# regeirk/pycwt

Hardware: NVIDIA H100
Metric: cwt_scale_points_per_sec (higher is better)
Workload: dtype f64

## Files before the change

### pycwt_b200/csrc/engine.cu

```cuda
#include <algorithm>
#include <array>
#include <cmath>
#include <cstdint>
#include <cstdio>
#include <cstdlib>
#include <cstring>
#include <map>
#include <mutex>
#include <set>
#include <string>
#include <type_traits>
#include <vector>

#include <cuda_runtime.h>
#include <dlfcn.h>
#include <initializer_list>

#include "../../include/cwt_b200.h"
#include "kernels.cuh"

using namespace cwtb;

template <class B, class = void> struct BodyNT { static constexpr int value = NT; };
template <class B> struct BodyNT<B, std::void_t<decltype(B::NTB)>> { static constexpr int value = B::NTB; };
// ... 100 lines not shown
  int log2K;
  int first, count;
  int expand = 0;
  int log2Nc = 0;
  int taps = 0;
  long long woff = 0;
  int os = 0;
};

struct ResidentSlot {
  Buf buf;
  int S = 0;
  long long n0 = 0;
  int prec = 0;
  long long serial = 0;
  Buf counts;
  long long units = -1;
};

static void slot_begin(ResidentSlot &s) {
  ++s.serial;
  s.S = 0;
  s.n0 = 0;
  s.units = -1;
}

struct OsRow { int grp = 0, t1 = 0, M = 0; long long hoff = 0; };

struct Job {
  bool valid = false;
  int precision = 0;
  long long n0 = 0;
  unsigned N = 0;
  int log2N = 0;
  int S = 0;
  int nbatch = 1;
  double dt = 0;
  Fam fam{};
  std::vector<ScaleDesc> descs;
  std::vector<ClassRun> classes;
  std::vector<int> plan_log2K;
  std::vector<double> scales;
  size_t b_single = 0;
  size_t coarse_elems = 0;
  int sig_is_f32 = 0;
  bool exact = false;
  std::vector<OsGroup> os_groups;
};

struct BluePlan {
  unsigned n = 0, L = 0;
  double2 *wm = nullptr;
  double2 *bf[2] = {nullptr, nullptr};
};

struct NTabDev {
  double2 *hi = nullptr, *lo = nullptr;
  int h = 0;
};

struct cwtb_ctx {
  int device = 0;
  rt_stream stream{};
  rt_stream aux_stream{};
  rt_stream prio_stream{};
  rt_stream prio_short{};
  int prio_mode = 1;
  rt_stream chain_streams[3]{};
  int n_chains = 2;
  rt_stream cur{};
  int pad_pow2 = 1;
  int coh_precision = 0;
  std::map<unsigned, BluePlan> blue;
  rt_stream copy_streams[2]{};
  std::string err;
  double band_eps = 1e-16;
  double band_eps32 = 1e-9;
  double expand_eps = 5e-13;
  double expand_eps32 = 2e-7;
  int expand_mma = 1;
  int dense_margin = 2;
  int expand_min_log2R = 0;
  int os_on = 1;
  Buf osH, osgrp;
  void *comm = nullptr;
  int comm_world = 1, comm_rank = 0;
  Buf comm_send, comm_recv;
  int group = 0;
  size_t group_bytes = (size_t)512 << 20;
  int num_sms = 132;
  int pf_dist = 132;
  int pf_rows_a = 32, pf_rows_b = 32;
  int pf_dist_a = 132;
  size_t batch_bytes = (size_t)4 << 30;
  double2 *tw64 = nullptr;
  float2 *tw32 = nullptr;
  std::map<unsigned, NTabDev> ntabs;
  Buf filt;
  int filt_rows = 0;
  long long filt_n = 0;
  Buf Zx, Cout, wtab;
  std::map<std::array<long long, 3>, long long> wtab_index;
  std::vector<double> wtab_host;
  size_t wtab_uploaded = 0;
  size_t wtab_max_bytes = (size_t)256 << 20;
  Buf sig, sig2, sig3, spec, Z, Zc[3], Y, B, W, W2, W3, descs, table, scratch, C, A12, F, aux, rowd, win, mask, hist, noise, wide, blueA, blueX, blueY, pspec, prot;
  Job job;
  struct PlanKey {
    long long n0 = -1;
    double dt = 0, param = 0, band_eps = 0, band_eps32 = 0, expand_eps = 0, expand_eps32 = 0;
    int S = 0, family = 0, precision = 0, nbatch = 0, pad = 0;
    std::vector<double> scales;
    bool operator==(const PlanKey &o) const {
      return n0 == o.n0 && dt == o.dt && param == o.param && band_eps == o.band_eps && band_eps32 == o.band_eps32 &&
             expand_eps == o.expand_eps && expand_eps32 == o.expand_eps32 && S == o.S && family == o.family &&
             precision == o.precision && nbatch == o.nbatch && pad == o.pad && scales == o.scales;
    }
  } plan_key;
  int plan_reuse = 1;
  void *stage_host[2] = {nullptr, nullptr};
  size_t stage_bytes = 0;
  Buf stage_dev[2], batch_power;
  int batch_pipeline = 1;
  double *angle_host = nullptr;
  ResidentSlot coh;
  ResidentSlot cross;
  ResidentSlot coh3;
  ResidentSlot wt;
  const void *job_dsig = nullptr;
  double last_ms = 0;
  int launches = 0;
  std::set<const void *> configured;
  bool profiling = false;
  const char *prof_tag = "";
  struct ProfRec { std::string name; unsigned gx, gy; int ev; };
  std::vector<ProfRec> prof;
  std::vector<rt_event> prof_events;
  std::set<void *> pinned, devallocs;
  rt_event e0{}, e1{};
  rt_event ev_fork{}, ev_join{}, ev_joinc[3]{}, ev_coarse{}, ev_coarse_short{};
  rt_event ev_h2d[2]{}, ev_used[2]{};
  rt_event ev_angle{};
};

static int fail(cwtb_ctx *c, int code, const std::string &msg) {
  if (c) c->err = msg;
  return code;
}
#define RT(call)                                                                             \
  do {                                                                                       \
    int e_ = (call);                                                                         \
    if (e_ != 0) return fail(c, CWTB_ERR_CUDA, std::string(#call) + ": " + rt_errstr(e_));   \
  } while (0)

static int ensure(cwtb_ctx *c, Buf &b, size_t bytes) {
  if (b.bytes >= bytes && b.p) return 0;
  if (b.p) rt_free(b.p);
  b.p = nullptr;
  b.bytes = 0;
  if (rt_malloc(&b.p, bytes) != 0) return fail(c, CWTB_ERR_NOMEM, "device allocation failed");
  b.bytes = bytes;
  return 0;
}

#ifdef CWTB_HOST_EMU
template <class Body, int PH>
static void emu_phases(const typename Body::Args &a, int bx, int by, void *sm) {
  for (int tid = 0; tid < BodyNT<Body>::value; ++tid) Body::template phase<PH>(a, bx, by, tid, sm);
  if constexpr (PH + 1 < Body::NPHASE) emu_phases<Body, PH + 1>(a, bx, by, sm);
}
#endif

static std::string body_name(const char *pretty) {
  std::string s(pretty);
  size_t i = s.find("Body = ");
  if (i == std::string::npos) return s;
  s = s.substr(i + 7);
  size_t j = s.find_first_of(";]");
  if (j != std::string::npos) s = s.substr(0, j);
  if (s.rfind("cwtb::", 0) == 0) s = s.substr(6);
  return s;
}

constexpr unsigned MAX_ROWS = 65535;

template <class Body, class Dispatch>
static int launch_rec(cwtb_ctx *c, unsigned gx, unsigned gy, Dispatch &&dispatch) {
  if (gx == 0 || gy == 0) return 0;
  if (gy > MAX_ROWS) return fail(c, CWTB_ERR_ARG, "too many rows in one launch");
  int ev = -1;
  if (c->profiling) {
    ev = (int)c->prof.size() * 2;
    while ((int)c->prof_events.size() < ev + 2) {
      rt_event e;
      RT(rt_event_create(&e));
      c->prof_events.push_back(e);
    }
    c->prof.push_back({std::string(c->prof_tag) + body_name(__PRETTY_FUNCTION__), gx, gy, ev});
    RT(rt_record(c->prof_events[ev], c->cur));
  }
  int e = dispatch();
  if (e) return e;
  if (ev >= 0) RT(rt_record(c->prof_events[ev + 1], c->cur));
  c->launches++;
  return 0;
}

template <class Body>
static int launch(cwtb_ctx *c, unsigned gx, unsigned gy, const typename Body::Args &a) {
  return launch_rec<Body>(c, gx, gy, [&]() -> int {
#ifdef CWTB_HOST_EMU
    std::vector<unsigned char> smv(Body::SMEM + 64);
    unsigned char *sm = smv.data();
    sm += (16 - ((unsigned long long)sm & 15)) & 15;
    for (unsigned by = 0; by < gy; ++by)
      for (unsigned bx = 0; bx < gx; ++bx) emu_phases<Body, 0>(a, (int)bx, (int)by, sm);
    if (emu_bulk_copy_faults() != 0) {
      emu_bulk_copy_faults() = 0;
      return fail(c, CWTB_ERR_CUDA, "emulation: bulk-async copy with a misaligned address or size");
    }
#else
    const void *fn = (const void *)k_run<Body>;
    if (Body::SMEM > 48 * 1024 && !c->configured.count(fn)) {
// ... 550 lines not shown
  for (int r0 = 0; r0 < nrows; r0 += chunk) {
    const int nr = std::min(chunk, nrows - r0);
    BluePreArgs pa{(const char *)in + (size_t)r0 * in_pitch * isz, (double2 *)c->blueA.p, pl->wm,
                   in_pitch, (long long)n, n, real_in, sign};
    if ((e = launch<BluePreBody>(c, (n + NT - 1) / NT, nr, pa))) return e;
    if ((e = blue_convolve(c, *pl, nr, sign))) return e;
    BluePostArgs po{(const double2 *)c->blueY.p, out, pl->wm, nullptr, out_pitch, nout,
                    scale / (double)pl->L, pl->L, 0, r0, sign, EPI_STORE};
    if ((e = launch<BluePostBody>(c, (unsigned)((nout + NT - 1) / NT), nr, po))) return e;
  }
  return 0;
}

static int run_job_exact(cwtb_ctx *c, const Job &job, const double *dsig, double2 *Wout, int epi) {
  const unsigned n = job.N;
  const int S = job.S;
  int e;
  if (job.nbatch != 1) return fail(c, CWTB_ERR_UNSUPPORTED, "batched transforms need the padded mode");
  if ((e = ensure(c, c->spec, (size_t)n * sizeof(double2)))) return e;
  if (!Wout) {
    if ((e = ensure(c, c->W, (size_t)S * job.n0 * sizeof(double2)))) return e;
    Wout = (double2 *)c->W.p;
  }
  if ((e = blue_rows(c, dsig, 1, n, (double2 *)c->spec.p, n, n, 1, -1, 1.0, n))) return e;
  const BluePlan *pl;
  if ((e = get_blue(c, n, &pl))) return e;
  Fam fam = job.fam;
  if (fam.family == CWTB_TABLE) fam.table = (const double2 *)c->table.p;
  const int chunk = blue_chunk_rows(pl->L, S);
  if ((e = ensure(c, c->blueA, (size_t)chunk * n * sizeof(double2)))) return e;
  if ((e = ensure(c, c->blueX, (size_t)chunk * pl->L * sizeof(double2)))) return e;
  if ((e = ensure(c, c->blueY, (size_t)chunk * pl->L * sizeof(double2)))) return e;
  const ScaleDesc *ddesc = (const ScaleDesc *)c->descs.p;
  for (int r0 = 0; r0 < S; r0 += chunk) {
    const int nr = std::min(chunk, S - r0);
    BlueProdArgs pa{ddesc, (const double2 *)c->spec.p, (double2 *)c->blueA.p, pl->wm, fam, (long long)n, n, r0};
    if ((e = launch<BlueProdBody>(c, (n + NT - 1) / NT, nr, pa))) return e;
    if ((e = blue_convolve(c, *pl, nr, +1))) return e;
    BluePostArgs po{(const double2 *)c->blueY.p, Wout, pl->wm, ddesc, job.n0, job.n0,
                    1.0 / (double)pl->L, pl->L, r0, 0, +1, epi};
    if ((e = launch<BluePostBody>(c, (unsigned)((job.n0 + NT - 1) / NT), nr, po))) return e;
  }
  return 0;
}

template <typename T, int K>
static int launch_single(cwtb_ctx *c, const SingleArgs<T> &a, int count) {
  constexpr int P = Lay<T, K>::P;
  const unsigned M = a.N / K;
  return launch<SingleBody<T, K>>(c, (M + P - 1) / P, count, a);
}

static int chunk_rows(const cwtb_ctx *c, unsigned N, size_t elem_bytes) {
  if (c->group > 0) return c->group;
  size_t g = c->group_bytes / ((size_t)N * elem_bytes);
  return (int)std::max<size_t>(1, std::min<size_t>(g, 32768));
}

static bool class_single(const Job &job, const ClassRun &cl) {
  return !cl.expand && !cl.os && (cl.log2K <= 10 || (cl.log2K <= DIRECT_MAX_LOG2 && cl.log2K < job.log2N));
}
static bool class_two_kernel(const Job &job, const ClassRun &cl) {
  return !cl.expand && !cl.os && !class_single(job, cl);
}

static int job_chain_region(const cwtb_ctx *c, const Job &job, const ClassRun &cl) {
  int idx = 0;
  for (const ClassRun &o : job.classes) {
    if (&o == &cl) break;
    if (class_two_kernel(job, o)) ++idx;
  }
  return idx % std::max(1, c->n_chains);
}

static size_t band_chunk_elems(const Job &job, int G) {
  size_t bchunk = 0;
  for (const ClassRun &cl : job.classes)
    if (class_two_kernel(job, cl) && cl.log2K < job.log2N)
      bchunk = std::max(bchunk, (size_t)std::min(G, cl.count) << cl.log2K);
  return bchunk;
}

#ifndef CWTB_HOST_EMU
template <class Body>
static int launch_persistent(cwtb_ctx *c, unsigned gm, unsigned rows, const typename Body::Args &a) {
  auto kern = k_persist<Body>;
  const void *fn = (const void *)kern;
  if (!c->configured.count(fn)) {
    RT(cudaFuncSetAttribute(kern, cudaFuncAttributeMaxDynamicSharedMemorySize, (int)Body::SMEM));
    c->configured.insert(fn);
  }
  int occ = 0;
  RT(cudaOccupancyMaxActiveBlocksPerMultiprocessor(&occ, kern, Body::NTB, Body::SMEM));
  if (occ < 1) return fail(c, CWTB_ERR_CUDA, "persistent kernel does not fit on an SM");
  const unsigned long long total = (unsigned long long)gm * rows;
  if (total > 0xffffffffull) return fail(c, CWTB_ERR_ARG, "too many tiles in one launch");
  const unsigned grid = (unsigned)std::min<unsigned long long>(total, (unsigned long long)occ * c->num_sms);
  return launch_rec<Body>(c, grid, rows, [&]() -> int {
    kern<<<grid, Body::NTB, Body::SMEM, c->cur>>>(a, gm, (unsigned)total);
    RT(cudaGetLastError());
    return 0;
  });
}
#endif

template <class Body, typename T>
static int launch_coarse(cwtb_ctx *c, CoarseArgs<T> a, const std::vector<CoarseSeg> &segs) {
  for (size_t s0 = 0; s0 < segs.size(); s0 += CSEG_MAX) {
    a.nseg = (int)std::min<size_t>(CSEG_MAX, segs.size() - s0);
    unsigned ctas = 0;
    for (int i = 0; i < a.nseg; ++i) {
      a.seg[i] = segs[s0 + i];
      a.seg[i].cta0 = (int)ctas;
      ctas += (unsigned)Body::ctas(a.seg[i].log2Nc, a.seg[i].count);
    }
    int e = launch<Body>(c, ctas, 1, a);
    if (e) return e;
  }
  return 0;
}

template <typename T, int TAPS>
static int launch_expand_t(cwtb_ctx *c, const ExpandArgs<T> &a, int rows, int min_log2Nc) {
  using B = ExpandBody<T, TAPS>;
  const unsigned gx = std::max<unsigned>(1, a.N / (unsigned)(B::NT * B::L));
#ifndef CWTB_HOST_EMU
  if constexpr (std::is_same<T, double>::value) {
    static_assert(ExpandMmaBody<TAPS>::OUT_PER_CTA == 4096, "the planner assumes the tensor-core kernel from Np = 2^12");
    if (c->expand_mma && a.N >= (unsigned)ExpandMmaBody<TAPS>::OUT_PER_CTA) {
      const unsigned gm = a.N / (32u * std::min<unsigned>(ExpandMmaBody<TAPS>::L, 1u << min_log2Nc));
      if (a.epi == EPI_MULCONJ) return launch_persistent<ExpandMmaBody<TAPS, EPI_MULCONJ>>(c, gm, rows, a);
      return launch_persistent<ExpandMmaBody<TAPS>>(c, gm, rows, a);
    }
  }
  if constexpr (TAPS > 16) {
    return fail(c, CWTB_ERR_STATE, "expansion: tap counts above 16 exist on the tensor-core kernel only");
  } else
#endif
  {
    if (a.epi == EPI_MULCONJ) return launch<ExpandBody<T, TAPS, EPI_MULCONJ>>(c, gx, rows, a);
    return launch<B>(c, gx, rows, a);
  }
}
template <typename T>
static int launch_expand(cwtb_ctx *c, int taps, const ExpandArgs<T> &a, int rows, int min_log2Nc) {
  if constexpr (std::is_same<T, double>::value) {
    switch (taps) {
      case 10: return launch_expand_t<T, 10>(c, a, rows, min_log2Nc);
      case 12: return launch_expand_t<T, 12>(c, a, rows, min_log2Nc);
      case 14: return launch_expand_t<T, 14>(c, a, rows, min_log2Nc);
      case 16: return launch_expand_t<T, 16>(c, a, rows, min_log2Nc);
      case 20: return launch_expand_t<T, 20>(c, a, rows, min_log2Nc);
    }
  } else {
    switch (taps) {
      case 6: return launch_expand_t<T, 6>(c, a, rows, min_log2Nc);
      case 8: return launch_expand_t<T, 8>(c, a, rows, min_log2Nc);
      case 10: return launch_expand_t<T, 10>(c, a, rows, min_log2Nc);
    }
  }
  return fail(c, CWTB_ERR_STATE, "expansion: unsupported tap count");
}

template <typename T>
static int run_job(cwtb_ctx *c, const Job &job, const T *dsig, cx<T> *Wout = nullptr, int epi = EPI_STORE) {
  using V = cx<T>;
  if (job.exact) {
    if constexpr (std::is_same<T, double>::value) return run_job_exact(c, job, dsig, Wout, epi);
    else return fail(c, CWTB_ERR_UNSUPPORTED, "un-padded transforms run in fp64");
  }
  const unsigned N = job.N;
  const int S = job.S * job.nbatch;
  int e;
  struct CurGuard { cwtb_ctx *c; ~CurGuard() { c->cur = c->stream; c->prof_tag = ""; } } cur_guard{c};
  if ((e = ensure(c, c->spec, (size_t)job.nbatch * N * sizeof(V)))) return e;
  if (!Wout) {
    if ((e = ensure(c, c->W, (size_t)S * job.n0 * sizeof(V)))) return e;
    Wout = (V *)c->W.p;
  }
  V *spec = (V *)c->spec.p;
  V *W = Wout;
  const ScaleDesc *ddesc = (const ScaleDesc *)c->descs.p;
  Fam fam = job.fam;
  if (fam.family == CWTB_TABLE) fam.table = (const double2 *)c->table.p;

  if (N < 32) {
    if (job.nbatch != 1) return fail(c, CWTB_ERR_UNSUPPORTED, "batched transform needs n0 > 16");
    TinyFwdArgs<T> fa{dsig, spec, job.n0, N};
    if ((e = launch<TinyFwdBody<T>>(c, 1, 1, fa))) return e;
    TinyArgs<T> ta{ddesc, spec, W, fam, job.n0, N, 0, epi};
    return launch<TinyBody<T>>(c, (unsigned)((job.n0 + NT - 1) / NT), S, ta);
  }
  c->prof_tag = "fwd:";
  e = fft_rows<T, -1>(c, dsig, 1, job.n0, job.n0, spec, N, N, job.nbatch);
  c->prof_tag = "";
  if (e) return e;

  NTab nt;
  if ((e = get_ntab(c, N, job.log2N, &nt))) return e;
  const int G = chunk_rows(c, N, sizeof(V));
  const size_t bchunk = band_chunk_elems(job, G);
  if ((e = ensure(c, c->B, (job.b_single + (size_t)std::max(1, c->n_chains) * bchunk) * sizeof(V)))) return e;
  V *Bbuf = (V *)c->B.p;

  {
    int first = -1, maxlk = 0, nrows = 0;
    for (const ClassRun &cl : job.classes)
      if (class_single(job, cl)) {
        if (first < 0) first = cl.first;
        maxlk = std::max(maxlk, cl.log2K);
        nrows += cl.count;
      }
    if (first >= 0) {
      BandArgs<T> ba{ddesc, spec, Bbuf, fam, N, first};
      const unsigned Kmax = 1u << maxlk;
      if ((e = launch<BandBody<T>>(c, (Kmax + NT * BandBody<T>::PER - 1) / (NT * BandBody<T>::PER), nrows, ba)))
        return e;
    }
  }
  const bool split = !c->profiling;
  if (split) {
    RT(rt_record(c->ev_fork, c->stream));
    RT(rt_wait(c->aux_stream, c->ev_fork));
    for (int k = 1; k < c->n_chains; ++k) RT(rt_wait(c->chain_streams[k - 1], c->ev_fork));
  }
  if (job.coarse_elems) {
    const bool prio = split && c->prio_mode > 0;
    if (prio) {
      RT(rt_wait(c->prio_stream, c->ev_fork));
      RT(rt_wait(c->prio_short, c->ev_fork));
    }
    if (split) c->cur = prio ? c->prio_stream : c->aux_stream;
    if ((e = ensure(c, c->Cout, job.coarse_elems * sizeof(V)))) return e;
    std::vector<CoarseSeg> short_segs, long_segs;
    size_t zx_elems = 0;
    for (size_t ci = 0; ci < job.classes.size(); ++ci) {
      const ClassRun &cl = job.classes[ci];
      if (!cl.expand) continue;
      if (cl.log2Nc < 6 || cl.log2Nc > 20)
        return fail(c, CWTB_ERR_STATE, "expansion: coarse length outside 2^6 .. 2^20");
      std::vector<CoarseSeg> &v = cl.log2Nc <= 10 ? short_segs : long_segs;
      if (ci > 0 && job.classes[ci - 1].expand && job.classes[ci - 1].log2Nc == cl.log2Nc) v.back().count += cl.count;
      else v.push_back(CoarseSeg{cl.first, cl.count, cl.log2Nc, 0});
      if (cl.log2Nc > 10)
        zx_elems = std::max(zx_elems, (size_t)job.descs[cl.first].ip_coff + ((size_t)cl.count << cl.log2Nc));
    }
    CoarseArgs<T> ca{};
    ca.descs = ddesc; ca.spec = spec; ca.C = (V *)c->Cout.p; ca.tw = Tw<T>::get(c); ca.fam = fam; ca.Nx = N;
    ca.pf_dist = c->pf_rows_b;
    c->prof_tag = "coarse:";
    if (!long_segs.empty()) {
      if ((e = ensure(c, c->Zx, zx_elems * sizeof(V)))) return e;
      ca.Z = (V *)c->Zx.p;
      for (const CoarseSeg &g : long_segs)
        if ((e = get_ntab(c, 1u << g.log2Nc, g.log2Nc, &ca.nt[g.log2Nc - 10]))) return e;
      if ((e = launch_coarse<CoarseABody<T>>(c, ca, long_segs))) return e;
      if ((e = launch_coarse<CoarseBBody<T>>(c, ca, long_segs))) return e;
    }
    if (!short_segs.empty()) {
      if (prio) c->cur = c->prio_short;
      if ((e = launch_coarse<CoarseRowsBody<T>>(c, ca, short_segs))) return e;
    }
    c->prof_tag = "";
    if (prio) {
      RT(rt_record(c->ev_coarse_short, c->prio_short));
      RT(rt_record(c->ev_coarse, c->prio_stream));
      c->cur = c->prio_mode == 1 ? c->aux_stream : c->prio_stream;
      RT(rt_wait(c->cur, c->ev_coarse_short));
    }
    for (int pass = 0; pass < 2 && !e; ++pass) {
      if (pass == 1 && prio && c->prio_mode == 1) RT(rt_wait(c->cur, c->ev_coarse));
      for (size_t ci = 0; ci < job.classes.size() && !e; ++ci) {
        const ClassRun &cl = job.classes[ci];
        if (!cl.expand || (ci > 0 && job.classes[ci - 1].expand && job.classes[ci - 1].taps == cl.taps)) continue;
        int rows = 0, minl = 30, maxl = 0;
        for (size_t cj = ci; cj < job.classes.size() && job.classes[cj].expand && job.classes[cj].taps == cl.taps; ++cj) {
          rows += job.classes[cj].count;
          minl = std::min(minl, job.classes[cj].log2Nc);
          maxl = std::max(maxl, job.classes[cj].log2Nc);
        }
        if ((maxl > 10) != (pass == 1)) continue;
        ExpandArgs<T> ea{ddesc, (const V *)c->Cout.p, (const double *)c->wtab.p, W, nt, job.n0, N, cl.first, epi,
                         job.log2N};
        e = launch_expand<T>(c, cl.taps, ea, rows, minl);
      }
    }
    if (prio && !e) {
      if (c->prio_mode == 2) RT(rt_record(c->ev_coarse, c->prio_stream));
      RT(rt_wait(c->aux_stream, c->ev_coarse));
    }
    c->cur = c->stream;
    if (e) return e;
  }
  if (!job.os_groups.empty()) {
    if constexpr (std::is_same<T, double>::value) {
      unsigned gx = 0;
      for (const OsGroup &g : job.os_groups)
        gx = std::max<unsigned>(gx, (unsigned)((job.n0 + (long long)g.hop * OsBody<4>::P - 1) /
                                               ((long long)g.hop * OsBody<4>::P)));
      OsArgs oa{ddesc, (const OsGroup *)c->osgrp.p, dsig, (const double2 *)c->osH.p, W, Tw<T>::get(c),
                job.n0, N, epi};
      if ((e = launch<OsBody<4>>(c, gx, (unsigned)job.os_groups.size(), oa))) return e;
    } else {
      return fail(c, CWTB_ERR_STATE, "overlap-save rows run in fp64 only");
    }
  }
  for (int pass = 0; pass < 2; ++pass)
  for (const ClassRun &cl : job.classes) {
    if (cl.expand || cl.os) continue;
    const unsigned K = 1u << cl.log2K;
    const bool single = class_single(job, cl);
    if (single != (pass == 0)) continue;
    if (single) {
      if (split) c->cur = c->aux_stream;
      SingleArgs<T> sa{ddesc, Bbuf, W, Tw<T>::get(c), nt, job.n0, N, cl.first, epi};
      switch (cl.log2K) {
        case 5: e = launch_single<T, 32>(c, sa, cl.count); break;
        case 6: e = launch_single<T, 64>(c, sa, cl.count); break;
        case 7: e = launch_single<T, 128>(c, sa, cl.count); break;
        case 8: e = launch_single<T, 256>(c, sa, cl.count); break;
        case 9: e = launch_single<T, 512>(c, sa, cl.count); break;
        case 10: e = launch_single<T, 1024>(c, sa, cl.count); break;
        case 11: e = launch<DirectBody<T, 2>>(c, (N / K2C + Lay<T, K2C>::P - 1) / Lay<T, K2C>::P, cl.count, sa); break;
        case 12: e = launch<DirectBody<T, 4>>(c, (N / K2C + Lay<T, K2C>::P - 1) / Lay<T, K2C>::P, cl.count, sa); break;
        case 13: e = launch<DirectBody<T, 8>>(c, (N / K2C + Lay<T, K2C>::P - 1) / Lay<T, K2C>::P, cl.count, sa); break;
        default: e = fail(c, CWTB_ERR_STATE, "bad single-kernel class");
      }
      c->cur = c->stream;
      if (e) return e;
      continue;
    }
    const bool dense = (cl.log2K == job.log2N);
    if (dense && job.log2N > 20) {
      const int l0 = job.log2N - 20;
      const unsigned Nsub = 1u << 20;
      const int gy = std::max<int>(1, (int)std::min<size_t>((size_t)cl.count, ((size_t)512 << 20) / ((size_t)N * sizeof(V))));
      if ((e = ensure(c, c->Y, (size_t)gy * N * sizeof(V)))) return e;
      for (int g0 = 0; g0 < cl.count; g0 += gy) {
        const int ng = std::min(gy, cl.count - g0);
        PassAArgs<T> a{};
        a.descs = ddesc; a.spec = spec; a.Bbuf = Bbuf; a.Z = (V *)c->Y.p; a.tw = Tw<T>::get(c);
        a.fam = fam; a.nt = nt; a.N = N; a.first = cl.first + g0; a.row0 = 0;
        a.pf_dist = 0; a.K2 = Nsub;
        if ((e = dispatch_passA<T, +1, MODE_DENSE>(c, l0, a, ng))) return e;
        if ((e = two_kernel_rows<T, +1>(c, c->Y.p, 0, Nsub, Nsub, W, job.n0, Nsub, ng << l0, job.n0, nullptr, 1.0,
                                         1 << l0, ddesc, cl.first + g0, 0, epi)))
          return e;
      }
      continue;
    }
    const int chain = split ? job_chain_region(c, job, cl) : 0;
    Buf &Zb = chain > 0 ? c->Zc[chain - 1] : c->Z;
    if ((e = ensure(c, Zb, (size_t)G * N * sizeof(V)))) return e;
    c->cur = chain > 0 ? c->chain_streams[chain - 1] : c->stream;
    for (int g0 = 0; g0 < cl.count; g0 += G) {
      const int ng = std::min(G, cl.count - g0);
      PassAArgs<T> a{};
      a.descs = ddesc; a.spec = spec; a.Bbuf = Bbuf; a.Z = (V *)Zb.p; a.tw = Tw<T>::get(c);
      a.fam = fam; a.nt = nt; a.N = N; a.first = cl.first + g0; a.row0 = 0;
      constexpr bool k512_ok = (Lay<T, 512, true>::PITCH * sizeof(V)) % 16 == 0;
      const int l2k = (dense || cl.log2K > 16 || !k512_ok) ? 10 : 9;
      a.pf_dist = c->pf_dist_a; a.K2 = 1u << l2k;
      PassBArgs<T> b{};
      b.Z = (const V *)Zb.p; b.out = W; b.tw = Tw<T>::get(c); b.descs = ddesc;
      b.pitch = job.n0; b.nout = job.n0; b.N = N; b.first = cl.first + g0; b.row0 = 0;
      b.epi = epi; b.grow = nullptr; b.post = 1.0;
      b.pf_dist = c->pf_dist; b.ny = ng;
      if (!dense) {
        BandArgs<T> ba{ddesc, spec, Bbuf, fam, N, cl.first + g0};
        if ((e = launch<BandBody<T>>(c, (K + NT * BandBody<T>::PER - 1) / (NT * BandBody<T>::PER), ng, ba)))
          return e;
      }
      e = dense ? dispatch_passA<T, +1, MODE_DENSE>(c, cl.log2K - l2k, a, ng)
                : dispatch_passA<T, +1, MODE_BAND>(c, cl.log2K - l2k, a, ng);
      if (e) return e;
      if constexpr (k512_ok) {
        if (l2k == 9)
          e = launch<PassBBody<T, +1, 512>>(c, (N / 512 + Lay<T, 512>::P - 1) / Lay<T, 512>::P, ng, b);
      }
      if (l2k != 9)
        e = launch<PassBBody<T, +1>>(c, (N / K2C + Lay<T, K2C>::P - 1) / Lay<T, K2C>::P, ng, b);
      if (e) return e;
    }
    c->cur = c->stream;
  }
  if (split) {
    RT(rt_record(c->ev_join, c->aux_stream));
    RT(rt_wait(c->stream, c->ev_join));
    for (int k = 1; k < c->n_chains; ++k) {
      RT(rt_record(c->ev_joinc[k - 1], c->chain_streams[k - 1]));
      RT(rt_wait(c->stream, c->ev_joinc[k - 1]));
    }
  }
  return 0;
}

static void assign_chunk_offsets(cwtb_ctx *c, Job &job) {
  const int G = chunk_rows(c, job.N, job.precision == CWTB_F64 ? sizeof(double2) : sizeof(float2));
  const size_t bchunk = band_chunk_elems(job, G);
  for (const ClassRun &cl : job.classes) {
    if (!class_two_kernel(job, cl) || cl.log2K == job.log2N) continue;
    const size_t region = (size_t)job_chain_region(c, job, cl) * bchunk;
    for (int i = 0; i < cl.count; ++i)
      job.descs[cl.first + i].boff =
          (long long)(job.b_single + region + (size_t)(i % G) * ((size_t)1 << cl.log2K));
  }
}

static int upload_descs(cwtb_ctx *c, Job &job) {
  assign_chunk_offsets(c, job);
  if (c->wtab_host.size() > c->wtab_uploaded) {
    const size_t bytes = c->wtab_host.size() * sizeof(double);
    if (c->wtab.bytes < bytes) {
      RT(rt_sync(c->stream));
      int e2 = ensure(c, c->wtab, std::max(bytes, (size_t)2 * c->wtab.bytes));
      if (e2) return e2;
      c->wtab_uploaded = 0;
    }
    RT(rt_h2d((char *)c->wtab.p + c->wtab_uploaded * sizeof(double), c->wtab_host.data() + c->wtab_uploaded,
              (c->wtab_host.size() - c->wtab_uploaded) * sizeof(double), c->stream));
    c->wtab_uploaded = c->wtab_host.size();
  }
  int e = ensure(c, c->descs, job.descs.size() * sizeof(ScaleDesc));
  if (e) return e;
  RT(rt_h2d(c->descs.p, job.descs.data(), job.descs.size() * sizeof(ScaleDesc), c->stream));
  RT(rt_sync(c->stream));
  return 0;
}

static int time_begin(cwtb_ctx *c) {
  RT(rt_record(c->e0, c->stream));
  return 0;
}
static int time_stop(cwtb_ctx *c) {
  RT(rt_record(c->e1, c->stream));
  return 0;
}
static int time_read(cwtb_ctx *c, double *ms) {
  float f = 0;
  RT(rt_elapsed_ms(&f, c->e0, c->e1));
  *ms = f;
  return 0;
}
static int time_end(cwtb_ctx *c, double *ms) {
  int e = time_stop(c);
  if (e) return e;
  RT(rt_event_sync(c->e1));
  return time_read(c, ms);
}

static void w_fill(cwtb_ctx *c) {
  c->wt.S = c->job.S * c->job.nbatch;
  c->wt.n0 = c->job.n0;
  c->wt.prec = c->job.precision;
}
static int w_kept(cwtb_ctx *c, int e) {
  if (e) c->wt.S = 0;
  return e;
}

static int timed_run(cwtb_ctx *c, const void *dsig, int iters, double *ms_out) {
  const Job &job = c->job;
  c->launches = 0;
  int e = time_begin(c);
  if (e) return e;
  for (int it = 0; it < iters; ++it) {
    e = job.precision == CWTB_F64 ? run_job<double>(c, job, (const double *)dsig)
                                  : run_job<float>(c, job, (const float *)dsig);
    if (e) return e;
  }
  double ms = 0;
  if ((e = time_end(c, &ms))) return e;
  if (ms_out) *ms_out = ms / iters;
  c->launches /= std::max(1, iters);
  w_fill(c);
  return 0;
}

template <typename TI, typename TO> struct CvtArgs { const TI *in; TO *out; long long n; };
template <typename TI, typename TO> struct CvtBody {
  using Args = CvtArgs<TI, TO>;
  static constexpr int NPHASE = 1;
  static constexpr size_t SMEM = 0;
  template <int PH> HD static void phase(const Args &a, int bx, int, int tid, void *) {
    long long i = (long long)bx * NT + tid;
    if (i < a.n) a.out[i] = (TO)a.in[i];
  }
};

extern "C" {

const char *cwtb_version(void) {
#ifdef CWTB_HOST_EMU
  return "cwt_b200 0.1 (host emulation build - tests only)";
#else
  return "cwt_b200 0.1 (sm_90a)";
#endif
}

int cwtb_device_count(void) {
  int n = 0;
  if (rt_device_count(&n) != 0) return 0;
  return n;
}

int cwtb_create(int device, cwtb_ctx **out) {
  if (!out) return CWTB_ERR_ARG;
  *out = nullptr;
  cwtb_ctx *c = new cwtb_ctx();
  c->device = device;
  if (rt_set_device(device) != 0) { delete c; return CWTB_ERR_CUDA; }
  if (rt_stream_create(&c->stream) != 0) { delete c; return CWTB_ERR_CUDA; }
  rt_event_create(&c->e0);
  rt_event_create(&c->e1);
  for (auto &st : c->copy_streams) rt_stream_create(&st);
  rt_stream_create(&c->aux_stream);
  rt_stream_create_highest({&c->prio_stream, &c->prio_short});
  rt_event_create_sync(&c->ev_angle);
  rt_event_create_sync(&c->ev_coarse);
  rt_event_create_sync(&c->ev_coarse_short);
  for (auto &ev : c->ev_h2d) rt_event_create_sync(&ev);
  for (auto &ev : c->ev_used) rt_event_create_sync(&ev);
  if (const char *g = getenv("CWTB_BATCH_PIPELINE")) c->batch_pipeline = atoi(g) != 0;
  if (const char *g = getenv("CWTB_PRIO")) c->prio_mode = std::min(2, std::max(0, atoi(g)));
  for (auto &st : c->chain_streams) rt_stream_create(&st);
  for (auto &ev : c->ev_joinc) rt_event_create_sync(&ev);
  rt_event_create_sync(&c->ev_fork);
  rt_event_create_sync(&c->ev_join);
  c->cur = c->stream;
  if (const char *g = getenv("CWTB_GROUP")) c->group = std::max(0, atoi(g));
  if (const char *g = getenv("CWTB_GROUP_MB")) c->group_bytes = (size_t)std::max(1, atoi(g)) << 20;
  if (const char *g = getenv("CWTB_BAND_EPS")) c->band_eps = atof(g);
  if (const char *g = getenv("CWTB_BAND_EPS32")) c->band_eps32 = atof(g);
  if (const char *g = getenv("CWTB_EXPAND_EPS")) c->expand_eps = std::max(0.0, atof(g));
  if (const char *g = getenv("CWTB_EXPAND_EPS32")) c->expand_eps32 = std::max(0.0, atof(g));
  if (const char *g = getenv("CWTB_EXPAND_MIN_R")) c->expand_min_log2R = std::min(14, std::max(2, atoi(g)));
  if (const char *g = getenv("CWTB_EXPAND_MMA")) c->expand_mma = atoi(g) != 0;
  if (const char *g = getenv("CWTB_OS")) c->os_on = atoi(g) != 0;
  if (const char *g = getenv("CWTB_WTAB_MB")) c->wtab_max_bytes = (size_t)std::max(0, atoi(g)) << 20;
  if (const char *g = getenv("CWTB_PLAN_REUSE")) c->plan_reuse = atoi(g) != 0;
  if (const char *g = getenv("CWTB_DENSE_MARGIN")) c->dense_margin = std::max(0, atoi(g));
  if (const char *g = getenv("CWTB_PF_DIST")) c->pf_dist = std::max(0, atoi(g));
  if (const char *g = getenv("CWTB_CHAINS")) c->n_chains = std::min(4, std::max(1, atoi(g)));
  if (const char *g = getenv("CWTB_FFT_PAD")) c->pad_pow2 = atoi(g) != 0;
  if (const char *g = getenv("CWTB_PF_ROWS_A")) c->pf_rows_a = std::max(0, atoi(g));
  if (const char *g = getenv("CWTB_PF_ROWS_B")) c->pf_rows_b = std::max(0, atoi(g));
  if (const char *g = getenv("CWTB_PF_DIST_A")) c->pf_dist_a = std::max(0, atoi(g));
  if (const char *g = getenv("CWTB_BATCH_MB")) c->batch_bytes = (size_t)std::max(1, atoi(g)) << 20;
  rt_sm_count(&c->num_sms, device);
  int e = init_tables(c);
  if (e == 0) e = rt_sync(c->stream) ? CWTB_ERR_CUDA : 0;
  if (e) { delete c; return e; }
  *out = c;
  return CWTB_OK;
}

void cwtb_destroy(cwtb_ctx *c) {
  if (!c) return;
  rt_set_device(c->device);
  rt_sync(c->stream);
  cwtb_comm_destroy(c);
  for (Buf *b : {&c->osH, &c->osgrp, &c->stage_dev[0], &c->stage_dev[1], &c->batch_power, &c->filt, &c->comm_send, &c->comm_recv, &c->Zx, &c->Cout, &c->wtab, &c->sig, &c->sig2, &c->sig3, &c->spec, &c->Z, &c->Zc[0], &c->Zc[1], &c->Zc[2], &c->Y, &c->B, &c->W, &c->W2, &c->W3, &c->descs, &c->table, &c->scratch,
                 &c->C, &c->A12, &c->F, &c->aux, &c->rowd, &c->win, &c->mask, &c->hist, &c->noise, &c->wide, &c->blueA, &c->blueX, &c->blueY, &c->pspec, &c->prot, &c->coh.buf, &c->cross.buf, &c->coh3.buf, &c->coh.counts, &c->coh3.counts})
    if (b->p) rt_free(b->p);
  for (auto &kv : c->ntabs) { rt_free(kv.second.hi); rt_free(kv.second.lo); }
  for (auto &kv : c->blue) { rt_free(kv.second.wm); rt_free(kv.second.bf[0]); rt_free(kv.second.bf[1]); }
  if (c->tw64) rt_free(c->tw64);
  if (c->tw32) rt_free(c->tw32);
  for (void *p : c->pinned) rt_host_free(p);
  for (void *p : c->devallocs) rt_free(p);
  rt_event_destroy(c->e0);
  rt_event_destroy(c->e1);
  rt_stream_destroy(c->stream);
  for (auto &st : c->copy_streams) rt_stream_destroy(st);
  rt_stream_destroy(c->aux_stream);
  rt_stream_destroy(c->prio_stream);
  rt_stream_destroy(c->prio_short);
  rt_event_destroy(c->ev_angle);
  rt_event_destroy(c->ev_coarse);
  rt_event_destroy(c->ev_coarse_short);
  for (auto &ev : c->ev_h2d) rt_event_destroy(ev);
  for (auto &ev : c->ev_used) rt_event_destroy(ev);
  for (void *p : c->stage_host) if (p) rt_host_free(p);
  for (auto &st : c->chain_streams) rt_stream_destroy(st);
  for (auto &ev : c->ev_joinc) rt_event_destroy(ev);
  rt_event_destroy(c->ev_fork);
  rt_event_destroy(c->ev_join);
  delete c;
}

const char *cwtb_last_error(cwtb_ctx *c) { return c ? c->err.c_str() : "null context"; }

int cwtb_set_band_eps(cwtb_ctx *c, double eps) {
  if (!c || !(eps >= 0) || eps >= 1e-6) return fail(c, CWTB_ERR_ARG, "band eps must be in [0, 1e-6)");
  c->band_eps = eps;
  return 0;
}

int cwtb_set_expand_eps(cwtb_ctx *c, double eps64, double eps32) {
  if (!c || !(eps64 >= 0) || !(eps32 >= 0) || eps64 > 1e-6 || eps32 > 1e-3)
    return fail(c, CWTB_ERR_ARG, "expansion tolerance must be in [0, 1e-6] (fp64) / [0, 1e-3] (fp32)");
  c->expand_eps = eps64;
  c->expand_eps32 = eps32;
  return 0;
}

int cwtb_host_alloc(cwtb_ctx *c, size_t bytes, void **out) {
  if (!c || !out) return CWTB_ERR_ARG;
  if (rt_host_alloc(out, bytes) != 0) return fail(c, CWTB_ERR_NOMEM, "pinned allocation failed");
  c->pinned.insert(*out);
  return 0;
}
int cwtb_host_free(cwtb_ctx *c, void *p) {
  if (!c || !c->pinned.count(p)) return CWTB_ERR_ARG;
  c->pinned.erase(p);
  rt_host_free(p);
  return 0;
}
int cwtb_dev_alloc(cwtb_ctx *c, size_t bytes, void **out) {
  if (!c || !out) return CWTB_ERR_ARG;
  if (rt_malloc(out, bytes) != 0) return fail(c, CWTB_ERR_NOMEM, "device allocation failed");
  c->devallocs.insert(*out);
  return 0;
}
int cwtb_dev_free(cwtb_ctx *c, void *p) {
  if (!c || !c->devallocs.count(p)) return CWTB_ERR_ARG;
  c->devallocs.erase(p);
  rt_free(p);
  return 0;
}
int cwtb_memcpy_h2d(cwtb_ctx *c, void *dst, const void *src, size_t bytes) {
  RT(rt_h2d(dst, src, bytes, c->stream));
  RT(rt_sync(c->stream));
  return 0;
}
int cwtb_memcpy_d2h(cwtb_ctx *c, void *dst, const void *src, size_t bytes) {
  RT(rt_d2h(dst, src, bytes, c->stream));
  RT(rt_sync(c->stream));
  return 0;
}
int cwtb_sync(cwtb_ctx *c) {
  RT(rt_sync(c->stream));
  return 0;
}

static const double kOsUs = 7.0;
static const double kTwoKernelUs = 23.5;

struct DevTmp {
  void *p = nullptr;
  ~DevTmp() { if (p) rt_free(p); }
};

static int os_plan(cwtb_ctx *c, const Job &job, double dt, int family, double param, std::vector<OsRow> &os) {
  constexpr int L = OsBody<4>::L, GR = 4;
  auto os_cheaper = [](int M) { return M <= L / 2 && kOsUs * L / (double)(L - M + 1) < kTwoKernelUs; };
  os.assign(job.S, OsRow());
  const unsigned N = job.N;
  if (!c->os_on || job.precision != CWTB_F64 || job.exact || family == CWTB_TABLE ||
      !(c->band_eps > 0) || !(c->expand_eps > 0) || N < 2u * L)
    return 0;
  const long long half = (long long)N / 2;
  std::vector<int> cand;
  std::vector<double> cs;
  for (const ScaleDesc &d : job.descs) {
    if (d.chan != 0 || d.k_hi < d.k_lo || d.k_lo <= -half || d.k_hi >= ((long long)N - 1) / 2) continue;
    if (d.ip_log2Nc || (d.log2K <= 10 || (d.log2K <= DIRECT_MAX_LOG2 && d.log2K < job.log2N))) continue;
    cand.push_back(d.row);
    cs.push_back(d.s);
  }
  if (cand.empty()) return 0;
  const int nc = (int)cand.size();
  const size_t wcap = (size_t)job.S * job.nbatch * job.n0;
  const int chunk = (int)std::max<size_t>(1, wcap / N);
  int e = ensure(c, c->W, std::max<size_t>((size_t)chunk * N, wcap) * sizeof(double2));
  if (e) return e;
  double2 *h = (double2 *)c->W.p;
  DevTmp dimp, part;
  if (rt_malloc(&dimp.p, (size_t)N * sizeof(double))) return fail(c, CWTB_ERR_NOMEM, "device allocation failed");
  {
    std::vector<double> delta(N, 0.0);
    delta[0] = 1.0;
    RT(rt_h2d(dimp.p, delta.data(), (size_t)N * sizeof(double), c->stream));
    RT(rt_sync(c->stream));
  }
  const int nblk = 64;
  if (rt_malloc(&part.p, (size_t)chunk * nblk * sizeof(double))) return fail(c, CWTB_ERR_NOMEM, "device allocation failed");
  std::vector<double> farmax(nc, 0.0);
  std::vector<double2> win((size_t)nc * 2 * L);
  for (int r0 = 0; r0 < nc; r0 += chunk) {
    const int nr = std::min(chunk, nc - r0);
    Job imp;
    const double xeps = c->expand_eps;
    c->expand_eps = 0;
    e = build_job(c, imp, (long long)N, dt, cs.data() + r0, nr, family, param, CWTB_F64, false, 1);
    c->expand_eps = xeps;
    if (e) return e;
    if ((e = upload_descs(c, imp))) return e;
    if ((e = run_job<double>(c, imp, (const double *)dimp.p, h, EPI_STORE))) return e;
    if (N > 2u * L) {
      AbsMaxArgs aa{h, (double *)part.p, (long long)N, (long long)L, (long long)N - L, nblk};
      if ((e = launch<AbsMaxBody>(c, nblk, nr, aa))) return e;
      std::vector<double> ph((size_t)nr * nblk);
      RT(rt_d2h(ph.data(), part.p, ph.size() * sizeof(double), c->stream));
      RT(rt_sync(c->stream));
      for (int r = 0; r < nr; ++r)
        for (int b = 0; b < nblk; ++b) farmax[r0 + r] = std::max(farmax[r0 + r], ph[(size_t)r * nblk + b]);
    }
    for (int r = 0; r < nr; ++r) {
      RT(rt_d2h(&win[(size_t)(r0 + r) * 2 * L], h + (size_t)r * N + (N - L), L * sizeof(double2), c->stream));
      RT(rt_d2h(&win[(size_t)(r0 + r) * 2 * L + L], h + (size_t)r * N, L * sizeof(double2), c->stream));
    }
    RT(rt_sync(c->stream));
  }
  struct Acc { int r, t0, t1; };
  std::vector<Acc> acc;
  std::vector<double> m(2 * L), pre(2 * L + 1);
  for (int r = 0; r < nc; ++r) {
    const double2 *w = &win[(size_t)r * 2 * L];
    double mx = farmax[r];
    for (int i = 0; i < 2 * L; ++i) mx = std::max(mx, std::max(std::fabs(w[i].x), std::fabs(w[i].y)));
    const double ulp = 2.220446049250313e-16 * mx;
    if (!(mx > 0) || farmax[r] > 128 * ulp) continue;
    const double floor_ = std::max(2 * farmax[r], 8 * ulp);
    double l1 = 0;
    pre[0] = 0;
    for (int i = 0; i < 2 * L; ++i) {
      const double a = std::hypot(w[i].x, w[i].y);
      l1 += a;
      m[i] = std::max(std::fabs(w[i].x), std::fabs(w[i].y)) > floor_ ? a : 0.0;
// ... 1846 lines not shown
```

Measured before the change: 113.6 billion.

## Co-schedule tensor-core expansion rows beside FFT/overlap-save launches

Splits the fp64 expansion launches into a background part that runs on the short-priority stream concurrently with overlap-save and dense FFT rows, and a remainder launched after the FFT streams finish. The background share is sized from a cost model of the FFT work. The persistent expansion grid is capped so each SM keeps room (registers, shared memory, threads) for one FFT CTA. Short coarse segments are launched first so expansion can start earlier. The aim is to fill idle SM capacity during FFT phases, at the cost of more event synchronisation and possibly slower expansion CTAs from the reduced occupancy.

Result: faster. 116.0 billion, median of 6 (+2.1%).

```diff
diff --git a/profiles/micro/cosched_rates.py b/profiles/micro/cosched_rates.py
--- /dev/null
+++ b/profiles/micro/cosched_rates.py
@@ -0,0 +1,148 @@
+import json
+import os
+import subprocess
+import sys
+import tempfile
+
+import numpy as np
+
+ROOT = os.path.dirname(os.path.dirname(os.path.dirname(os.path.abspath(__file__))))
+sys.path.insert(0, ROOT)
+sys.path.insert(0, os.path.dirname(os.path.abspath(__file__)))
+import workloads as wl
+from pycwt_b200 import _engine
+from coarse_timeline import kind
+
+C = wl.C2
+
+
+def engine(env, x, sj):
+    old = {k: os.environ.get(k) for k in env}
+    os.environ.update({k: str(v) for k, v in env.items()})
+    try:
+        eng = _engine.Engine(0)
+    finally:
+        for k, v in old.items():
+            if v is None:
+                os.environ.pop(k, None)
+            else:
+                os.environ[k] = v
+    d = eng.dev_alloc(x.nbytes)
+    eng.h2d(d, x)
+    eng.cwt_dev(d, 0, C["n"], C["dt"], sj, _engine.MORLET, C["f0"], _engine.F64)
+    eng.bench_last(10)
+    eng._d = d
+    return eng
+
+
+def close(eng):
+    eng.dev_free(eng._d)
+    eng.close()
+
+
+def expand_rows(prof):
+    out = {}
+    for k in prof:
+        if k["name"].startswith("ExpandMmaBody<"):
+            taps = int(k["name"][len("ExpandMmaBody<"):].split(",")[0].rstrip(">"))
+            ms, rows = out.get(taps, (0.0, 0))
+            out[taps] = (ms + k["ms"], rows + k["rows"])
+    return out
+
+
+def timeline(eng, path):
+    from torch.profiler import ProfilerActivity, profile
+    eng.sync()
+    with profile(activities=[ProfilerActivity.CUDA]) as prof:
+        eng.bench_last(1)
+        eng.sync()
+    prof.export_chrome_trace(path)
+    with open(path) as f:
+        ev = [e for e in json.load(f)["traceEvents"] if e.get("cat") == "kernel"]
+    ev.sort(key=lambda e: e["ts"])
+    t0 = ev[0]["ts"]
+    k = [(kind(e["name"]), (e["ts"] - t0) / 1e3, (e["ts"] + e["dur"] - t0) / 1e3, e["name"]) for e in ev]
+    print("  step span %.3f ms, %d kernels" % (max(r[2] for r in k), len(k)))
+    for r in k:
+        if r[0] in ("expand", "os", "dense"):
+            print("    %-7s %.3f .. %.3f  (%.3f ms)  %s" % (r[0], r[1], r[2], r[2] - r[1], r[3][:90]))
+    ex = [r for r in k if r[0] == "expand"]
+    fb = [r for r in k if r[0] in ("os", "dense")]
+    ov = sum(max(0.0, min(a[2], b[2]) - max(a[1], b[1])) for a in ex for b in fb)
+    print("  overlap-save / dense launches overlapping an expansion launch: %.3f ms (sum over pairs)" % ov)
+
+
+def main():
+    args = [a for a in sys.argv[1:]]
+    rows = [0, 40, 60, 80, 100, 120]
+    rounds = 4
+    if "--rows" in args:
+        rows = [int(v) for v in args[args.index("--rows") + 1].split(",")]
+        del args[args.index("--rows"):args.index("--rows") + 2]
+    if "--rounds" in args:
+        rounds = int(args[args.index("--rounds") + 1])
+        del args[args.index("--rounds"):args.index("--rounds") + 2]
+    out_dir = args[0] if args else os.path.join(tempfile.gettempdir(), "cosched")
+    os.makedirs(out_dir, exist_ok=True)
+    import torch
+    torch.zeros(1, device="cuda")
+    print(subprocess.run(["nvidia-smi", "--query-gpu=name,power.limit,clocks.max.sm", "--format=csv"],
+                         capture_output=True, text=True).stdout.strip())
+    x = wl.config2_signal()
+    sj = wl.config2_scales()
+    n0 = C["n"]
+
+    print("1. expansion launches alone (serialised), grid capped at k CTAs per SM")
+    for k in (1, 2, 3, 4, 5):
+        eng = engine({"CWTB_COSCHED": 0, "CWTB_EXPAND_CTAS": k}, x, sj)
+        ms = []
+        for _ in range(5):
+            eng.bench_last(1)
+            ms.append(expand_rows(eng.profile_last()))
+        for taps in sorted(ms[0]):
+            t = float(np.median([m[taps][0] for m in ms]))
+            r = ms[0][taps][1]
+            print("  k=%d  ExpandMmaBody<%d>  %3d rows  %.4f ms  %5.2f us/row  W %.2f TB/s"
+                  % (k, taps, r, t, 1e3 * t / r, r * n0 * 16 / (t * 1e-3) / 1e12))
+        close(eng)
+
+    print("2. config 2 step, ms per step over %d runs of 20 steps: median (min-max)" % rounds)
+    arms = {"off": {"CWTB_COSCHED": 0}, "default": {"CWTB_COSCHED": 1}}
+    for r in rows:
+        arms["rows=%d" % r] = {"CWTB_COSCHED": 1, "CWTB_COSCHED_ROWS": r}
+    engs = {name: engine(env, x, sj) for name, env in arms.items()}
+    t = {name: [] for name in engs}
+    for _ in range(rounds):
+        for name, eng in engs.items():
+            t[name].append(eng.bench_last(20))
+    for name in engs:
+        print("  %-10s %.4f (%.4f-%.4f)" % (name, float(np.median(t[name])), min(t[name]), max(t[name])))
+    on = engs.pop("default")
+    off = engs.pop("off")
+    for eng in engs.values():
+        close(eng)
+
+    print("3. timeline of one step")
+    for name, eng in (("CWTB_COSCHED=0", off), ("CWTB_COSCHED=1", on)):
+        print(" " + name)
+        timeline(eng, os.path.join(out_dir, "cosched_%s.pt.trace.json" % name[-1]))
+    prof = on.profile_last()
+    print("  serialised, CWTB_COSCHED=1: " + ", ".join(
+        "%s %d rows" % (k["name"], k["rows"]) for k in prof if k["name"].startswith("ExpandMmaBody")))
+
+    print("4. W of the two schedules")
+    plan_on, plan_off = on.last_plan(len(sj)), off.last_plan(len(sj))
+    same = 0
+    for r0 in range(0, len(sj), 32):
+        a = np.empty((32, n0), np.complex128)
+        b = np.empty((32, n0), np.complex128)
+        on._check(on.lib.cwtb_get_w(on.h, _engine._ptr(a), 1, r0, 32))
+        off._check(off.lib.cwtb_get_w(off.h, _engine._ptr(b), 1, r0, 32))
+        same += sum(np.array_equal(a[i].view(np.uint64), b[i].view(np.uint64)) for i in range(32))
+    print("  plans identical: %s; rows bit-identical: %d of %d" % (list(plan_on) == list(plan_off), same, len(sj)))
+    close(on)
+    close(off)
+
+
+if __name__ == "__main__":
+    main()
diff --git a/pycwt_b200/csrc/engine.cu b/pycwt_b200/csrc/engine.cu
--- a/pycwt_b200/csrc/engine.cu
+++ b/pycwt_b200/csrc/engine.cu
@@ -206,6 +206,10 @@
   int dense_margin = 2;
   int expand_min_log2R = 0;
   int os_on = 1;
+  int cosched = 1;
+  int cosched_min_log2N = 20;
+  int cosched_rows = -1;
+  int expand_ctas = 0;
   Buf osH, osgrp;
   void *comm = nullptr;
   int comm_world = 1, comm_rank = 0;
@@ -263,6 +267,8 @@
   std::set<void *> pinned, devallocs;
   rt_event e0{}, e1{};
   rt_event ev_fork{}, ev_join{}, ev_joinc[3]{}, ev_coarse{}, ev_coarse_short{};
+  rt_event ev_fftb[4]{};
+  rt_event ev_xjoin{};
   rt_event ev_h2d[2]{}, ev_used[2]{};
   rt_event ev_angle{};
 };
@@ -979,8 +985,42 @@
 }
 
 #ifndef CWTB_HOST_EMU
+struct CtaUse { long long regs, smem, threads; };
+static int cta_use(cwtb_ctx *c, const void *fn, int ntb, size_t dyn_smem, CtaUse *u) {
+  cudaFuncAttributes fa;
+  RT(cudaFuncGetAttributes(&fa, fn));
+  int reserved = 0;
+  RT(cudaDeviceGetAttribute(&reserved, cudaDevAttrReservedSharedMemoryPerBlock, c->device));
+  const long long warps = (ntb + 31) / 32;
+  u->regs = warps * (((long long)fa.numRegs * 32 + 255) / 256 * 256);
+  u->smem = (long long)fa.sharedSizeBytes + (long long)dyn_smem + reserved;
+  u->threads = warps * 32;
+  return 0;
+}
+
 template <class Body>
-static int launch_persistent(cwtb_ctx *c, unsigned gm, unsigned rows, const typename Body::Args &a) {
+static int beside_fft_ctas(cwtb_ctx *c, const void *kern, int occ, int *out) {
+  int regs_sm = 0, smem_sm = 0, thr_sm = 0;
+  RT(cudaDeviceGetAttribute(&regs_sm, cudaDevAttrMaxRegistersPerMultiprocessor, c->device));
+  RT(cudaDeviceGetAttribute(&smem_sm, cudaDevAttrMaxSharedMemoryPerMultiprocessor, c->device));
+  RT(cudaDeviceGetAttribute(&thr_sm, cudaDevAttrMaxThreadsPerMultiProcessor, c->device));
+  CtaUse ex, os, dense;
+  using Dense = PassABody<double, 1024, MODE_DENSE, +1>;
+  int e = cta_use(c, kern, Body::NTB, Body::SMEM, &ex);
+  if (!e) e = cta_use(c, (const void *)k_run<OsBody<4>>, OsBody<4>::NTB, OsBody<4>::SMEM, &os);
+  if (!e) e = cta_use(c, (const void *)k_run<Dense>, Dense::NTB, Dense::SMEM, &dense);
+  if (e) return e;
+  int k = occ;
+  for (const CtaUse &f : {os, dense})
+    while (k > 1 && (k * ex.regs + f.regs > regs_sm || k * ex.smem + f.smem > smem_sm ||
+                     k * ex.threads + f.threads > thr_sm))
+      --k;
+  *out = k;
+  return 0;
+}
+
+template <class Body>
+static int launch_persistent(cwtb_ctx *c, unsigned gm, unsigned rows, const typename Body::Args &a, bool beside) {
   auto kern = k_persist<Body>;
   const void *fn = (const void *)kern;
   if (!c->configured.count(fn)) {
@@ -990,6 +1030,11 @@
   int occ = 0;
   RT(cudaOccupancyMaxActiveBlocksPerMultiprocessor(&occ, kern, Body::NTB, Body::SMEM));
   if (occ < 1) return fail(c, CWTB_ERR_CUDA, "persistent kernel does not fit on an SM");
+  if (beside) {
+    int e = beside_fft_ctas<Body>(c, fn, occ, &occ);
+    if (e) return e;
+  }
+  if (c->expand_ctas > 0) occ = std::min(occ, c->expand_ctas);
   const unsigned long long total = (unsigned long long)gm * rows;
   if (total > 0xffffffffull) return fail(c, CWTB_ERR_ARG, "too many tiles in one launch");
   const unsigned grid = (unsigned)std::min<unsigned long long>(total, (unsigned long long)occ * c->num_sms);
@@ -1018,7 +1063,7 @@
 }
 
 template <typename T, int TAPS>
-static int launch_expand_t(cwtb_ctx *c, const ExpandArgs<T> &a, int rows, int min_log2Nc) {
+static int launch_expand_t(cwtb_ctx *c, const ExpandArgs<T> &a, int rows, int min_log2Nc, bool beside) {
   using B = ExpandBody<T, TAPS>;
   const unsigned gx = std::max<unsigned>(1, a.N / (unsigned)(B::NT * B::L));
 #ifndef CWTB_HOST_EMU
@@ -1026,8 +1071,8 @@
     static_assert(ExpandMmaBody<TAPS>::OUT_PER_CTA == 4096, "the planner assumes the tensor-core kernel from Np = 2^12");
     if (c->expand_mma && a.N >= (unsigned)ExpandMmaBody<TAPS>::OUT_PER_CTA) {
       const unsigned gm = a.N / (32u * std::min<unsigned>(ExpandMmaBody<TAPS>::L, 1u << min_log2Nc));
-      if (a.epi == EPI_MULCONJ) return launch_persistent<ExpandMmaBody<TAPS, EPI_MULCONJ>>(c, gm, rows, a);
-      return launch_persistent<ExpandMmaBody<TAPS>>(c, gm, rows, a);
+      if (a.epi == EPI_MULCONJ) return launch_persistent<ExpandMmaBody<TAPS, EPI_MULCONJ>>(c, gm, rows, a, beside);
+      return launch_persistent<ExpandMmaBody<TAPS>>(c, gm, rows, a, beside);
     }
   }
   if constexpr (TAPS > 16) {
@@ -1040,23 +1085,36 @@
   }
 }
 template <typename T>
-static int launch_expand(cwtb_ctx *c, int taps, const ExpandArgs<T> &a, int rows, int min_log2Nc) {
+static int launch_expand(cwtb_ctx *c, int taps, const ExpandArgs<T> &a, int rows, int min_log2Nc, bool beside = false) {
   if constexpr (std::is_same<T, double>::value) {
     switch (taps) {
-      case 10: return launch_expand_t<T, 10>(c, a, rows, min_log2Nc);
-      case 12: return launch_expand_t<T, 12>(c, a, rows, min_log2Nc);
-      case 14: return launch_expand_t<T, 14>(c, a, rows, min_log2Nc);
-      case 16: return launch_expand_t<T, 16>(c, a, rows, min_log2Nc);
-      case 20: return launch_expand_t<T, 20>(c, a, rows, min_log2Nc);
+      case 10: return launch_expand_t<T, 10>(c, a, rows, min_log2Nc, beside);
+      case 12: return launch_expand_t<T, 12>(c, a, rows, min_log2Nc, beside);
+      case 14: return launch_expand_t<T, 14>(c, a, rows, min_log2Nc, beside);
+      case 16: return launch_expand_t<T, 16>(c, a, rows, min_log2Nc, beside);
+      case 20: return launch_expand_t<T, 20>(c, a, rows, min_log2Nc, beside);
     }
   } else {
     switch (taps) {
-      case 6: return launch_expand_t<T, 6>(c, a, rows, min_log2Nc);
-      case 8: return launch_expand_t<T, 8>(c, a, rows, min_log2Nc);
-      case 10: return launch_expand_t<T, 10>(c, a, rows, min_log2Nc);
+      case 6: return launch_expand_t<T, 6>(c, a, rows, min_log2Nc, beside);
+      case 8: return launch_expand_t<T, 8>(c, a, rows, min_log2Nc, beside);
+      case 10: return launch_expand_t<T, 10>(c, a, rows, min_log2Nc, beside);
     }
   }
   return fail(c, CWTB_ERR_STATE, "expansion: unsupported tap count");
+}
+
+static const double kOsUs = 7.0;
+static const double kTwoKernelUs = 23.5;
+
+static const double kCoExpandUs = 10.0;
+static int cosched_bg_rows(const cwtb_ctx *c, const Job &job) {
+  if (c->cosched_rows >= 0) return c->cosched_rows;
+  double us = 0;
+  for (const OsGroup &g : job.os_groups) us += g.count * kOsUs * OsBody<4>::L / g.hop;
+  for (const ClassRun &cl : job.classes)
+    if (class_two_kernel(job, cl)) us += cl.count * kTwoKernelUs * 0.5 * (1.0 + std::ldexp(1.0, cl.log2K - job.log2N));
+  return (int)(us / kCoExpandUs);
 }
 
 template <typename T>
@@ -1121,8 +1179,38 @@
     RT(rt_wait(c->aux_stream, c->ev_fork));
     for (int k = 1; k < c->n_chains; ++k) RT(rt_wait(c->chain_streams[k - 1], c->ev_fork));
   }
+  const bool prio = split && c->prio_mode > 0;
+  bool fft_rows = !job.os_groups.empty();
+  for (const ClassRun &cl : job.classes) fft_rows = fft_rows || class_two_kernel(job, cl);
+  const bool cosched = std::is_same<T, double>::value && c->cosched && job.log2N >= c->cosched_min_log2N &&
+                       c->expand_mma && job.coarse_elems && fft_rows;
+  const int bg_rows = cosched ? cosched_bg_rows(c, job) : 0;
+  auto expand_part = [&](int part) -> int {
+    int left = bg_rows;
+    for (int pass = 0; pass < 2; ++pass) {
+      if (pass == 1 && prio && (c->prio_mode == 1 || cosched)) RT(rt_wait(c->cur, c->ev_coarse));
+      for (size_t ci = 0; ci < job.classes.size(); ++ci) {
+        const ClassRun &cl = job.classes[ci];
+        if (!cl.expand || (ci > 0 && job.classes[ci - 1].expand && job.classes[ci - 1].taps == cl.taps)) continue;
+        int rows = 0, minl = 30, maxl = 0;
+        for (size_t cj = ci; cj < job.classes.size() && job.classes[cj].expand && job.classes[cj].taps == cl.taps; ++cj) {
+          rows += job.classes[cj].count;
+          minl = std::min(minl, job.classes[cj].log2Nc);
+          maxl = std::max(maxl, job.classes[cj].log2Nc);
+        }
+        if ((maxl > 10) != (pass == 1)) continue;
+        const int nbg = std::min(rows, left);
+        left -= nbg;
+        const int r0 = part == 2 ? nbg : 0, nr = part == 0 ? rows : part == 1 ? nbg : rows - nbg;
+        ExpandArgs<T> ea{ddesc, (const V *)c->Cout.p, (const double *)c->wtab.p, W, nt, job.n0, N, cl.first + r0,
+                         epi, job.log2N};
+        const int e = launch_expand<T>(c, cl.taps, ea, nr, minl, cosched && split);
+        if (e) return e;
+      }
+    }
+    return 0;
+  };
   if (job.coarse_elems) {
-    const bool prio = split && c->prio_mode > 0;
     if (prio) {
       RT(rt_wait(c->prio_stream, c->ev_fork));
       RT(rt_wait(c->prio_short, c->ev_fork));
@@ -1146,6 +1234,12 @@
     ca.descs = ddesc; ca.spec = spec; ca.C = (V *)c->Cout.p; ca.tw = Tw<T>::get(c); ca.fam = fam; ca.Nx = N;
     ca.pf_dist = c->pf_rows_b;
     c->prof_tag = "coarse:";
+    const bool short_first = cosched && prio;
+    if (short_first && !short_segs.empty()) {
+      c->cur = c->prio_short;
+      if ((e = launch_coarse<CoarseRowsBody<T>>(c, ca, short_segs))) return e;
+      c->cur = c->prio_stream;
+    }
     if (!long_segs.empty()) {
       if ((e = ensure(c, c->Zx, zx_elems * sizeof(V)))) return e;
       ca.Z = (V *)c->Zx.p;
@@ -1154,7 +1248,7 @@
       if ((e = launch_coarse<CoarseABody<T>>(c, ca, long_segs))) return e;
       if ((e = launch_coarse<CoarseBBody<T>>(c, ca, long_segs))) return e;
     }
-    if (!short_segs.empty()) {
+    if (!short_first && !short_segs.empty()) {
       if (prio) c->cur = c->prio_short;
       if ((e = launch_coarse<CoarseRowsBody<T>>(c, ca, short_segs))) return e;
     }
@@ -1165,23 +1259,8 @@
       c->cur = c->prio_mode == 1 ? c->aux_stream : c->prio_stream;
       RT(rt_wait(c->cur, c->ev_coarse_short));
     }
-    for (int pass = 0; pass < 2 && !e; ++pass) {
-      if (pass == 1 && prio && c->prio_mode == 1) RT(rt_wait(c->cur, c->ev_coarse));
-      for (size_t ci = 0; ci < job.classes.size() && !e; ++ci) {
-        const ClassRun &cl = job.classes[ci];
-        if (!cl.expand || (ci > 0 && job.classes[ci - 1].expand && job.classes[ci - 1].taps == cl.taps)) continue;
-        int rows = 0, minl = 30, maxl = 0;
-        for (size_t cj = ci; cj < job.classes.size() && job.classes[cj].expand && job.classes[cj].taps == cl.taps; ++cj) {
-          rows += job.classes[cj].count;
-          minl = std::min(minl, job.classes[cj].log2Nc);
-          maxl = std::max(maxl, job.classes[cj].log2Nc);
-        }
-        if ((maxl > 10) != (pass == 1)) continue;
-        ExpandArgs<T> ea{ddesc, (const V *)c->Cout.p, (const double *)c->wtab.p, W, nt, job.n0, N, cl.first, epi,
-                         job.log2N};
-        e = launch_expand<T>(c, cl.taps, ea, rows, minl);
-      }
-    }
+    if (cosched && prio) c->cur = c->prio_short;
+    e = expand_part(cosched ? 1 : 0);
     if (prio && !e) {
       if (c->prio_mode == 2) RT(rt_record(c->ev_coarse, c->prio_stream));
       RT(rt_wait(c->aux_stream, c->ev_coarse));
@@ -1281,6 +1360,21 @@
     }
     c->cur = c->stream;
   }
+  if (cosched) {
+    if (split) {
+      c->cur = prio ? c->prio_short : c->aux_stream;
+      for (int k = 0; k < std::max(1, c->n_chains); ++k) {
+        RT(rt_record(c->ev_fftb[k], k ? c->chain_streams[k - 1] : c->stream));
+        RT(rt_wait(c->cur, c->ev_fftb[k]));
+      }
+    }
+    if ((e = expand_part(2))) return e;
+    if (prio) {
+      RT(rt_record(c->ev_xjoin, c->prio_short));
+      RT(rt_wait(c->aux_stream, c->ev_xjoin));
+    }
+    c->cur = c->stream;
+  }
   if (split) {
     RT(rt_record(c->ev_join, c->aux_stream));
     RT(rt_wait(c->stream, c->ev_join));
@@ -1424,6 +1518,8 @@
   for (auto &ev : c->ev_joinc) rt_event_create_sync(&ev);
   rt_event_create_sync(&c->ev_fork);
   rt_event_create_sync(&c->ev_join);
+  for (auto &ev : c->ev_fftb) rt_event_create_sync(&ev);
+  rt_event_create_sync(&c->ev_xjoin);
   c->cur = c->stream;
   if (const char *g = getenv("CWTB_GROUP")) c->group = std::max(0, atoi(g));
   if (const char *g = getenv("CWTB_GROUP_MB")) c->group_bytes = (size_t)std::max(1, atoi(g)) << 20;
@@ -1434,6 +1530,10 @@
   if (const char *g = getenv("CWTB_EXPAND_MIN_R")) c->expand_min_log2R = std::min(14, std::max(2, atoi(g)));
   if (const char *g = getenv("CWTB_EXPAND_MMA")) c->expand_mma = atoi(g) != 0;
   if (const char *g = getenv("CWTB_OS")) c->os_on = atoi(g) != 0;
+  if (const char *g = getenv("CWTB_COSCHED")) c->cosched = atoi(g) != 0;
+  if (const char *g = getenv("CWTB_COSCHED_MIN_LOG2N")) c->cosched_min_log2N = std::max(0, atoi(g));
+  if (const char *g = getenv("CWTB_COSCHED_ROWS")) c->cosched_rows = std::max(0, atoi(g));
+  if (const char *g = getenv("CWTB_EXPAND_CTAS")) c->expand_ctas = std::max(0, atoi(g));
   if (const char *g = getenv("CWTB_WTAB_MB")) c->wtab_max_bytes = (size_t)std::max(0, atoi(g)) << 20;
   if (const char *g = getenv("CWTB_PLAN_REUSE")) c->plan_reuse = atoi(g) != 0;
   if (const char *g = getenv("CWTB_DENSE_MARGIN")) c->dense_margin = std::max(0, atoi(g));
@@ -1483,6 +1583,8 @@
   for (auto &ev : c->ev_joinc) rt_event_destroy(ev);
   rt_event_destroy(c->ev_fork);
   rt_event_destroy(c->ev_join);
+  for (auto &ev : c->ev_fftb) rt_event_destroy(ev);
+  rt_event_destroy(c->ev_xjoin);
   delete c;
 }
 
@@ -1540,9 +1642,6 @@
   RT(rt_sync(c->stream));
   return 0;
 }
-
-static const double kOsUs = 7.0;
-static const double kTwoKernelUs = 23.5;
 
 struct DevTmp {
   void *p = nullptr;
```
